# imulki/serenade

Hardware: AMD Instinct MI355X
Metric: mel frames/sec converted (UNet ODE + vocoder), 80x1024 (higher is better)
Workload: dtype f32

## Files before the change

### include/serenade_hip.h

```cpp
#ifndef SERENADE_HIP_H
#define SERENADE_HIP_H

#include <stdint.h>

#ifdef __cplusplus
extern "C" {
#endif

#define SRN_ABI_VERSION 4
#define SRN_MAX_TAPS 16

enum { SRN_ACT_NONE = 0, SRN_ACT_LEAKY = 1, SRN_ACT_SILU = 2, SRN_ACT_MISH = 3 };
enum { SRN_RES_NONE = 0, SRN_RES_ADD = 1, SRN_RES_AXPY = 2 };
enum {
  SRN_POST_NONE = 0,
  SRN_POST_DIV = 1,
  SRN_POST_TANH = 2,
  SRN_POST_RELU = 3,
  SRN_POST_LEAKY = 4,
  SRN_POST_GELU = 5
};
enum {
  SRN_PREC_FP32 = 0,
  SRN_PREC_BF16X3 = 1,
  SRN_PREC_BF16X6 = 2
};
enum {
  SRN_ROUTE_AUTO = 0,
  SRN_ROUTE_TILED = 1,
  SRN_ROUTE_HALO = 2,
  SRN_ROUTE_GENERIC = 3,
  SRN_ROUTE_STRIP = 4,
  SRN_ROUTE_FAST_FP32 = 5
};
enum {
  SRN_FAMILY_GENERIC = 0,
  SRN_FAMILY_F32 = 1,
  SRN_FAMILY_FAST = 2,
  SRN_FAMILY_HALO = 3,
  SRN_FAMILY_STRIP = 4
};

typedef struct SrnConvParams {
  int32_t n_batch;
  int32_t n_head;
  int32_t T_in, T_out;
  int32_t C_in;
  int32_t C_in0;
  int32_t C_w;
  int32_t N;
  int32_t N_out;
  int32_t n_taps;
  int32_t tap_off[SRN_MAX_TAPS];
  int32_t in_stride;
  int32_t pad_reflect;
  int32_t w_nmajor;
  int32_t pro_act;
  float pro_slope;
  float alpha;
  float beta;
  int32_t geglu;
  int32_t res_mode;
  int32_t post;
  float post_div;
  int32_t out_t_stride, out_t_off;
  int32_t tile;
  const float* in0; int64_t in0_bs, in0_hs; int32_t ld_in0;
  const float* in1; int64_t in1_bs; int32_t ld_in1;
  const float* w;   int64_t w_bs, w_hs; int32_t ldw;
  const float* bias;
  const int32_t* len_in;
  const int32_t* len_out;
  const float* res;  int64_t res_bs, res_hs; int32_t ld_res;
  const float* res2; int64_t res2_bs; int32_t ld_res2;
  float* out; int64_t out_bs, out_hs; int32_t ld_out;
  int32_t precision;
  int32_t route;
  void* ws; int64_t ws_bytes;
  const void* w_hi; const void* w_lo;
  float* gn_partials;
  float* out_tr; int64_t out_tr_bs; int32_t ld_out_tr; int32_t out_tr_col0;
} SrnConvParams;

int srn_abi_version(void);
const char* srn_last_error(void);

int srn_conv_gemm(const SrnConvParams* p, void* stream);
int64_t srn_conv_gemm_workspace_bytes(const SrnConvParams* p);
int srn_conv_gemm_route(const SrnConvParams* p, int32_t out[3]);
#define SRN_FORM_FIELDS 9
int srn_conv_gemm_forms(int32_t* rows, int capacity);

int srn_gn_mish_apply(const float* x, const float* gn_partials, const float* gamma, const float* beta,
                      const float* time_bias, int64_t time_bias_bs, const int32_t* lens, float* y, int B, int T,
                      int C, int groups, float eps, int valid_stats, void* stream);

int srn_resblock_tail(const float* c2, const float* gn_partials, const float* gamma, const float* beta,
                      const int32_t* lens, const float* r, const float* scale, const float* shift, int64_t ld_ss,
                      float* y, int B, int T, int C, int groups, float gn_eps, float ln_eps, int valid_stats,
                      void* stream);

int srn_resblock_tail_ln(const float* c2, const float* gn_partials, const float* gamma, const float* beta,
                         const int32_t* lens, const float* r, const float* scale, const float* shift, int64_t ld_ss,
                         float* y, int B, int T, int C, int groups, float gn_eps, float ln_eps, int valid_stats,
                         const float* ln2_gamma, const float* ln2_beta, float* y2, float ln2_eps, void* stream);

int srn_layernorm(const float* x, const float* gamma, const float* beta, float* y, int64_t rows, int C, float eps,
                  void* stream);

int srn_softmax_rows(float* s, const int32_t* lens, int Z, int n_head, int L, int ld, void* stream);

int srn_sinusoidal_emb(const float* t, float* out, int n, int dim, int ld, float scale, void* stream);

int srn_copy_channels(const float* src, int64_t src_bs, int ld_src, int sc0, float* dst, int64_t dst_bs, int ld_dst,
                      int dc0, int B, int T, int C, void* stream);

int srn_scatter_rows(const float* src, int64_t src_bs, int ld_src, float* dst, int64_t dst_bs, int ld_dst, int dc0,
                     const int32_t* row_off, const int32_t* n_rows, int B, int T, int C, void* stream);

int srn_transpose_ct(const float* src, float* dst, int B, int R, int Cc, int64_t src_bs, int ld_src, int64_t dst_bs,
                     int ld_dst, void* stream);
#define SRN_TR_LIST_MAX 40
typedef struct SrnTransposeList {
  int32_t n;
  int32_t pad_;
  const float* src[SRN_TR_LIST_MAX];
  float* dst[SRN_TR_LIST_MAX];
  int64_t src_bs[SRN_TR_LIST_MAX], dst_bs[SRN_TR_LIST_MAX];
  int32_t B[SRN_TR_LIST_MAX], R[SRN_TR_LIST_MAX], Cc[SRN_TR_LIST_MAX];
  int32_t ld_src[SRN_TR_LIST_MAX], ld_dst[SRN_TR_LIST_MAX];
  int32_t first_block[SRN_TR_LIST_MAX + 1];
} SrnTransposeList;
int srn_transpose_multi(const SrnTransposeList* list, void* stream);

int srn_renorm(const float* x, const float* trg_scale, const float* trg_mean, const float* voc_mean,
               const float* voc_scale, float* y, int64_t rows, int C, void* stream);

int srn_out_conv_tanh(const float* x, const float* w, const float* bias, float* y, int B, int T, int C, int k,
                      float slope, void* stream);

typedef struct SrnResUnitParams {
  int32_t n_batch, T, C;
  int32_t k, dilation;
  float slope;
  const float* x; int64_t x_bs;
  const float* w1; const float* b1; const float* w2; const float* b2;
  const void* w1_hi; const void* w2_hi;
  const float* res2; int64_t res2_bs;
  float post_div;
  float* out; int64_t out_bs;
  int32_t precision;
  int32_t route;
} SrnResUnitParams;
enum { SRN_RESUNIT_ROUTE_SHARED = 1 };


int srn_hifigan_resunit(const SrnResUnitParams* p, void* stream);
enum { SRN_RESUNIT_FORM_F32 = 0, SRN_RESUNIT_FORM_SHARED_F32 = 1, SRN_RESUNIT_FORM_BF16X3 = 2 };
int srn_hifigan_resunit_route(const SrnResUnitParams* p, int32_t out[3]);

int srn_pd_gather(const float* x, const float* d, float* out, int B, int T, int C, float dilation, float slope,
                  void* stream);

int srn_gru_recur_last(const float* gi, const float* w_hh_t, const float* b_hh, float* h, int B, int T, int H,
                       void* stream);

int srn_style_token_attention_kv(const float* ref, const float* wq_t, const float* bq, const float* k, const float* v,
                                 const float* wo_t, const float* bo, float* out, int B, int Dq, int n_tok, int F,
                                 int n_head, void* stream);

int srn_pad_signal(const float* x, float* out, int B, int n, int pad, int ld, int mode, void* stream);
int srn_logmel(const float* spec, const float* mel_t, float* out, int64_t frames, int n_bins, int ld, int n_mels,
               float eps, int log_mode, void* stream);
int srn_loudness(const float* spec, const float* a_weight_db, uint32_t* gmax_ws, float* out, int B, int frames,
                 int n_bins, int ld, float amin, float top_db, float add_eps, void* stream);
int srn_pad_ragged_zero(const float* x, int64_t x_bs, const int32_t* lens, float* out, int B, int n, int pad, int ld,
                        void* stream);
int srn_logmel_ragged(const float* spec, const float* mel_t, const int32_t* frames, float* out, int B, int T,
                      int n_bins, int ld, int n_mels, float eps, int log_mode, void* stream);
int srn_loudness_ragged(const float* spec, const float* a_weight_db, const int32_t* frames, uint32_t* gmax_ws,
                        float* out, int B, int T, int n_bins, int ld, float amin, float top_db, float add_eps,
                        void* stream);

int srn_rowln_fwd(const float* x, const float* m, int64_t m_bs, const float* a, int64_t a_bs, float* y, int B, int T,
                  int C, float eps, void* stream);
int srn_rowln_bwd(const float* x, const float* dy, const float* m, int64_t m_bs, float* dx, float* partial, int B, int T,
                  int C, float eps, void* stream);
int srn_rowln_chunks(int T);
int srn_gn_mish_bwd_partial(const float* h, const float* dy, const float* mean, const float* rstd, const float* gamma,
                            const float* beta, const int32_t* lens, float* partial, int B, int T, int C, int groups,
                            void* stream);
int srn_gn_mish_bwd_apply(const float* h, const float* dy, const float* mean, const float* rstd, const float* gamma,
                          const float* beta, const float* gsum, const int32_t* lens, float* dh, int B, int T, int C,
                          int groups, void* stream);
int srn_gn_chunks(int T);
int srn_gn_stats(const float* partials, float* mean, float* rstd, int B, int T, int C, int groups, float eps,
                 void* stream);
int srn_chunk_colsum(const float* partial, const float* gamma, float* col, float* gsum, int B, int n_chunk, int C,
                     int groups, void* stream);
int srn_colsum(const float* x, float* partial, float* out, int B, int64_t R, int N, int ld, void* stream);
int srn_colsum_chunks(int64_t R);
int srn_softmax_bwd(const float* p, float* dp, int64_t rows, int L, int ld, float scale, void* stream);
int srn_geglu_fwd(const float* hg, float* a, int64_t rows, int inner, void* stream);
int srn_geglu_bwd(const float* hg, const float* da, float* dhg, int64_t rows, int inner, void* stream);
int srn_adamw(float* p, const float* g, float* m, float* v, int64_t n, float lr, float beta1, float beta2, float eps,
              float weight_decay, int step, float grad_scale, void* stream);
int srn_adamw_dyn(float* p, const float* g, float* m, float* v, int64_t n, float beta1, float beta2, float eps,
                  float weight_decay, const float* dyn, void* stream);
int srn_sumsq(const float* g, int64_t n, double* partial, void* stream);
int srn_dot(const float* a, const float* b, int64_t n, double* partial, void* stream);
#define SRN_COPY_LIST_MAX 160
typedef struct SrnCopyList {
  int32_t n;
  int32_t pad_;
  const void* src[SRN_COPY_LIST_MAX];
  int64_t off[SRN_COPY_LIST_MAX];
  int64_t len[SRN_COPY_LIST_MAX];
} SrnCopyList;
int srn_multi_copy(const SrnCopyList* list, float* dst, void* stream);
int srn_sumsq_blocks(int64_t n);
int srn_weight_norm_fwd(const float* v, const float* g, float* w_packed, float* wd, float* inv_norm, int N, int C, int k,
                        void* stream);
int srn_weight_norm_bwd(const float* dw_packed, const float* v, const float* g, const float* inv_norm, float* dv,
                        float* dg, int N, int C, int k, void* stream);

typedef struct SrnWorldParams {
  int32_t n_batch, max_frames;
  int32_t fs, fft_size;
  const double* x; int64_t x_bs; const int32_t* x_len;
  const double* f0; const double* t; int64_t f_bs;
  const int32_t* n_frames;
  const double* twiddle;
  double q1, f0_floor;
  double threshold;
  double unvoiced_db;
  const double* band_window; int32_t band_window_len;
  int32_t n_bands;
  double* out0; int64_t out0_bs; int32_t ld_out0;
  double* out1; int64_t out1_bs; int32_t ld_out1;
} SrnWorldParams;
int srn_world_cheaptrick(const SrnWorldParams* p, void* stream);
int srn_world_d4c(const SrnWorldParams* p, void* stream);
int srn_world_project(const double* in, int64_t rows, int K, int ld_in, const double* mat_t, int n_out, int take_log,
                      double* out, int ld_out, void* stream);
int srn_world_pack_features(const double* a, int na, const double* b, int nb, const double* mean, const double* scale,
                            float* out, int64_t rows, int ld_out, void* stream);
int srn_wave_to_f64(const float* wave, double* out, int64_t n, int pcm16, void* stream);
int srn_f0_match_length(const double* in, int64_t in_bs, const int32_t* n_in, double* out, int64_t out_bs,
// ... 136 lines not shown
```

### serenade_amd/_lib.py

```python
import collections
import ctypes
import os
from ctypes import POINTER, c_char_p, c_double, c_float, c_int, c_int32, c_int64, c_void_p

_HERE = os.path.dirname(os.path.abspath(__file__))
LIB_PATH = os.environ.get("SERENADE_AMD_LIB") or os.path.join(_HERE, "libserenade_hip.so")

SRN_MAX_TAPS = 16
ACT_NONE, ACT_LEAKY, ACT_SILU, ACT_MISH = 0, 1, 2, 3
RES_NONE, RES_ADD, RES_AXPY = 0, 1, 2
POST_NONE, POST_DIV, POST_TANH, POST_RELU, POST_LEAKY, POST_GELU = 0, 1, 2, 3, 4, 5
PREC_FP32, PREC_BF16X3, PREC_BF16X6 = 0, 1, 2
ROUTE_AUTO, ROUTE_TILED, ROUTE_HALO, ROUTE_GENERIC, ROUTE_STRIP, ROUTE_FAST_FP32 = 0, 1, 2, 3, 4, 5
FAMILY_GENERIC, FAMILY_F32, FAMILY_FAST, FAMILY_HALO, FAMILY_STRIP = 0, 1, 2, 3, 4
RESUNIT_ROUTE_SHARED = 1
TN_ROUTE_GENERAL = 1
RESUNIT_FORM_F32, RESUNIT_FORM_SHARED_F32, RESUNIT_FORM_BF16X3 = 0, 1, 2


class SrnConvParams(ctypes.Structure):
    _fields_ = [
        ("n_batch", c_int32), ("n_head", c_int32), ("T_in", c_int32), ("T_out", c_int32),
        ("C_in", c_int32), ("C_in0", c_int32), ("C_w", c_int32), ("N", c_int32), ("N_out", c_int32),
        ("n_taps", c_int32), ("tap_off", c_int32 * SRN_MAX_TAPS), ("in_stride", c_int32),
        ("pad_reflect", c_int32), ("w_nmajor", c_int32), ("pro_act", c_int32), ("pro_slope", c_float),
        ("alpha", c_float), ("beta", c_float), ("geglu", c_int32), ("res_mode", c_int32), ("post", c_int32), ("post_div", c_float),
        ("out_t_stride", c_int32), ("out_t_off", c_int32), ("tile", c_int32),
        ("in0", c_void_p), ("in0_bs", c_int64), ("in0_hs", c_int64), ("ld_in0", c_int32),
        ("in1", c_void_p), ("in1_bs", c_int64), ("ld_in1", c_int32),
        ("w", c_void_p), ("w_bs", c_int64), ("w_hs", c_int64), ("ldw", c_int32),
        ("bias", c_void_p), ("len_in", c_void_p), ("len_out", c_void_p),
        ("res", c_void_p), ("res_bs", c_int64), ("res_hs", c_int64), ("ld_res", c_int32),
        ("res2", c_void_p), ("res2_bs", c_int64), ("ld_res2", c_int32),
        ("out", c_void_p), ("out_bs", c_int64), ("out_hs", c_int64), ("ld_out", c_int32),
        ("precision", c_int32), ("route", c_int32), ("ws", c_void_p), ("ws_bytes", c_int64),
        ("w_hi", c_void_p), ("w_lo", c_void_p), ("gn_partials", c_void_p),
        ("out_tr", c_void_p), ("out_tr_bs", c_int64), ("ld_out_tr", c_int32), ("out_tr_col0", c_int32),
    ]


class SrnResUnitParams(ctypes.Structure):
    _fields_ = [
        ("n_batch", c_int32), ("T", c_int32), ("C", c_int32), ("k", c_int32), ("dilation", c_int32),
        ("slope", c_float), ("x", c_void_p), ("x_bs", c_int64),
        ("w1", c_void_p), ("b1", c_void_p), ("w2", c_void_p), ("b2", c_void_p),
        ("w1_hi", c_void_p), ("w2_hi", c_void_p), ("res2", c_void_p), ("res2_bs", c_int64),
        ("post_div", c_float), ("out", c_void_p), ("out_bs", c_int64), ("precision", c_int32), ("route", c_int32),
    ]


SRN_COPY_LIST_MAX = 160


class SrnCopyList(ctypes.Structure):
    _fields_ = [("n", c_int32), ("pad_", c_int32), ("src", c_void_p * SRN_COPY_LIST_MAX),
                ("off", c_int64 * SRN_COPY_LIST_MAX), ("len", c_int64 * SRN_COPY_LIST_MAX)]


class SrnWorldParams(ctypes.Structure):
    _fields_ = [
        ("n_batch", c_int32), ("max_frames", c_int32), ("fs", c_int32), ("fft_size", c_int32),
        ("x", c_void_p), ("x_bs", c_int64), ("x_len", c_void_p),
        ("f0", c_void_p), ("t", c_void_p), ("f_bs", c_int64), ("n_frames", c_void_p), ("twiddle", c_void_p),
        ("q1", c_double), ("f0_floor", c_double), ("threshold", c_double), ("unvoiced_db", c_double),
        ("band_window", c_void_p), ("band_window_len", c_int32), ("n_bands", c_int32),
        ("out0", c_void_p), ("out0_bs", c_int64), ("ld_out0", c_int32),
        ("out1", c_void_p), ("out1_bs", c_int64), ("ld_out1", c_int32),
    ]


SRN_TR_LIST_MAX = 40


class SrnTransposeList(ctypes.Structure):
    _fields_ = [("n", c_int32), ("pad_", c_int32), ("src", c_void_p * SRN_TR_LIST_MAX), ("dst", c_void_p * SRN_TR_LIST_MAX),
                ("src_bs", c_int64 * SRN_TR_LIST_MAX), ("dst_bs", c_int64 * SRN_TR_LIST_MAX),
                ("B", c_int32 * SRN_TR_LIST_MAX), ("R", c_int32 * SRN_TR_LIST_MAX), ("Cc", c_int32 * SRN_TR_LIST_MAX),
                ("ld_src", c_int32 * SRN_TR_LIST_MAX), ("ld_dst", c_int32 * SRN_TR_LIST_MAX),
                ("first_block", c_int32 * (SRN_TR_LIST_MAX + 1))]


class SrnTnGemmParams(ctypes.Structure):
    _fields_ = [
        ("n_batch", c_int32), ("n_head", c_int32), ("n_items", c_int32), ("T_a", c_int32), ("T_b", c_int32),
        ("stride", c_int32), ("n_shifts", c_int32), ("shift", c_int32 * SRN_MAX_TAPS), ("M", c_int32), ("N", c_int32),
        ("a", c_void_p), ("a_bs", c_int64), ("a_hs", c_int64), ("a_is", c_int64), ("lda", c_int32),
        ("b", c_void_p), ("b_bs", c_int64), ("b_hs", c_int64), ("b_is", c_int64), ("ldb", c_int32),
        ("out", c_void_p), ("out_bs", c_int64), ("out_hs", c_int64), ("ldc", c_int32),
        ("alpha", c_float), ("ws", c_void_p), ("ws_bytes", c_int64),
        ("n_inner", c_int32), ("a_is2", c_int64), ("b_is2", c_int64), ("len_b", c_void_p), ("colsum", c_void_p),
        ("route", c_int32),
    ]


class SrnExcitationParams(ctypes.Structure):
    _fields_ = [
        ("n_batch", c_int32), ("max_frames", c_int32), ("fs", c_int32), ("hop", c_int32),
        ("f0", c_void_p), ("df_f0", c_void_p), ("f_bs", c_int64), ("n_frames", c_void_p), ("phase_ws", c_void_p),
        ("noise", c_void_p), ("sine", c_void_p), ("sine_amp", c_float), ("noise_amp", c_float), ("n_df", c_int32),
        ("dfs", c_void_p * 4), ("df_upsample", c_int32 * 4), ("dense_factors", c_double * 4),
    ]


_P = c_void_p
_SIGS = {
    "srn_abi_version": (c_int, []),
    "srn_last_error": (c_char_p, []),
    "srn_conv_gemm": (c_int, [POINTER(SrnConvParams), _P]),
    "srn_conv_gemm_workspace_bytes": (c_int64, [POINTER(SrnConvParams)]),
    "srn_conv_gemm_route": (c_int, [POINTER(SrnConvParams), POINTER(c_int32)]),
    "srn_conv_gemm_forms": (c_int, [POINTER(c_int32), c_int]),
    "srn_hifigan_resunit": (c_int, [POINTER(SrnResUnitParams), _P]),
    "srn_hifigan_resunit_route": (c_int, [POINTER(SrnResUnitParams), POINTER(c_int32)]),
    "srn_gn_mish_apply": (c_int, [_P, _P, _P, _P, _P, c_int64, _P, _P, c_int, c_int, c_int, c_int, c_float, c_int, _P]),
    "srn_resblock_tail": (c_int, [_P, _P, _P, _P, _P, _P, _P, _P, c_int64, _P, c_int, c_int, c_int, c_int,
                                  c_float, c_float, c_int, _P]),
    "srn_resblock_tail_ln": (c_int, [_P, _P, _P, _P, _P, _P, _P, _P, c_int64, _P, c_int, c_int, c_int, c_int,
                                     c_float, c_float, c_int, _P, _P, _P, c_float, _P]),
    "srn_scatter_rows": (c_int, [_P, c_int64, c_int, _P, c_int64, c_int, c_int, _P, _P, c_int, c_int, c_int, _P]),
    "srn_layernorm": (c_int, [_P, _P, _P, _P, c_int64, c_int, c_float, _P]),
    "srn_softmax_rows": (c_int, [_P, _P, c_int, c_int, c_int, c_int, _P]),
    "srn_sinusoidal_emb": (c_int, [_P, _P, c_int, c_int, c_int, c_float, _P]),
    "srn_copy_channels": (c_int, [_P, c_int64, c_int, c_int, _P, c_int64, c_int, c_int, c_int, c_int, c_int, _P]),
    "srn_transpose_ct": (c_int, [_P, _P, c_int, c_int, c_int, c_int64, c_int, c_int64, c_int, _P]),
    "srn_transpose_multi": (c_int, [POINTER(SrnTransposeList), _P]),
    "srn_weight_norm_fwd": (c_int, [_P, _P, _P, _P, _P, c_int, c_int, c_int, _P]),
    "srn_weight_norm_bwd": (c_int, [_P, _P, _P, _P, _P, _P, c_int, c_int, c_int, _P]),
    "srn_renorm": (c_int, [_P, _P, _P, _P, _P, _P, c_int64, c_int, _P]),
    "srn_out_conv_tanh": (c_int, [_P, _P, _P, _P, c_int, c_int, c_int, c_int, c_float, _P]),
    "srn_pd_gather": (c_int, [_P, _P, _P, c_int, c_int, c_int, c_float, c_float, _P]),
    "srn_pad_signal": (c_int, [_P, _P, c_int, c_int, c_int, c_int, c_int, _P]),
    "srn_logmel": (c_int, [_P, _P, _P, c_int64, c_int, c_int, c_int, c_float, c_int, _P]),
    "srn_loudness": (c_int, [_P, _P, _P, _P, c_int, c_int, c_int, c_int, c_float, c_float, c_float, _P]),
    "srn_pad_ragged_zero": (c_int, [_P, c_int64, _P, _P, c_int, c_int, c_int, c_int, _P]),
    "srn_logmel_ragged": (c_int, [_P, _P, _P, _P, c_int, c_int, c_int, c_int, c_int, c_float, c_int, _P]),
    "srn_loudness_ragged": (c_int, [_P, _P, _P, _P, _P, c_int, c_int, c_int, c_int, c_float, c_float, c_float, _P]),
    "srn_gru_recur_last": (c_int, [_P, _P, _P, _P, c_int, c_int, c_int, _P]),
    "srn_style_token_attention_kv": (c_int, [_P] * 8 + [c_int] * 5 + [_P]),
    "srn_rowln_fwd": (c_int, [_P, _P, c_int64, _P, c_int64, _P, c_int, c_int, c_int, c_float, _P]),
    "srn_rowln_bwd": (c_int, [_P, _P, _P, c_int64, _P, _P, c_int, c_int, c_int, c_float, _P]),
    "srn_rowln_chunks": (c_int, [c_int]),
    "srn_gn_mish_bwd_partial": (c_int, [_P] * 8 + [c_int] * 4 + [_P]),
    "srn_gn_mish_bwd_apply": (c_int, [_P] * 9 + [c_int] * 4 + [_P]),
    "srn_gn_chunks": (c_int, [c_int]),
    "srn_gn_stats": (c_int, [_P, _P, _P, c_int, c_int, c_int, c_int, c_float, _P]),
    "srn_chunk_colsum": (c_int, [_P, _P, _P, _P, c_int, c_int, c_int, c_int, _P]),
    "srn_colsum": (c_int, [_P, _P, _P, c_int, c_int64, c_int, c_int, _P]),
    "srn_colsum_chunks": (c_int, [c_int64]),
    "srn_softmax_bwd": (c_int, [_P, _P, c_int64, c_int, c_int, c_float, _P]),
    "srn_geglu_fwd": (c_int, [_P, _P, c_int64, c_int, _P]),
    "srn_geglu_bwd": (c_int, [_P, _P, _P, c_int64, c_int, _P]),
    "srn_adamw": (c_int, [_P, _P, _P, _P, c_int64, c_float, c_float, c_float, c_float, c_float, c_int, c_float, _P]),
    "srn_adamw_dyn": (c_int, [_P, _P, _P, _P, c_int64, c_float, c_float, c_float, c_float, _P, _P]),
    "srn_sumsq": (c_int, [_P, c_int64, _P, _P]),
    "srn_dot": (c_int, [_P, _P, c_int64, _P, _P]),
    "srn_multi_copy": (c_int, [POINTER(SrnCopyList), _P, _P]),
    "srn_sumsq_blocks": (c_int, [c_int64]),
    "srn_bn_chunks": (c_int, [c_int64]),
    "srn_bn_relu_fwd": (c_int, [_P] * 8 + [c_int64, c_int, c_float, c_float, _P]),
    "srn_bn_relu_bwd": (c_int, [_P] * 8 + [c_int64, c_int, _P]),
    "srn_im2col_s2": (c_int, [_P, _P] + [c_int] * 5 + [_P]),
    "srn_col2im_s2": (c_int, [_P, _P] + [c_int] * 5 + [_P]),
    "srn_gru_train_fwd": (c_int, [_P] * 5 + [c_int] * 3 + [_P]),
    "srn_gru_train_bwd": (c_int, [_P] * 6 + [c_int] * 3 + [_P]),
    "srn_token_attn_fwd": (c_int, [_P] * 5 + [c_int] * 4 + [_P]),
    "srn_token_attn_bwd": (c_int, [_P] * 8 + [c_int] * 4 + [_P]),
    "srn_tn_gemm": (c_int, [POINTER(SrnTnGemmParams), _P]),
    "srn_tn_gemm_workspace_bytes": (c_int64, [POINTER(SrnTnGemmParams)]),
    "srn_tn_gemm_route": (c_int, [POINTER(SrnTnGemmParams), POINTER(c_int32)]),
    "srn_world_cheaptrick": (c_int, [POINTER(SrnWorldParams), _P]),
    "srn_world_d4c": (c_int, [POINTER(SrnWorldParams), _P]),
    "srn_world_project": (c_int, [_P, c_int64, c_int, c_int, _P, c_int, c_int, _P, c_int, _P]),
    "srn_world_pack_features": (c_int, [_P, c_int, _P, c_int, _P, _P, _P, c_int64, c_int, _P]),
    "srn_wave_to_f64": (c_int, [_P, _P, c_int64, c_int, _P]),
    "srn_f0_match_length": (c_int, [_P, c_int64, _P, _P, c_int64, _P, c_int, c_int, _P]),
    "srn_cont_f0": (c_int, [_P, c_int64, _P, _P, _P, _P, c_int, _P]),
    "srn_sifigan_excitation": (c_int, [POINTER(SrnExcitationParams), _P]),
    "srn_frame_stats_chunks": (c_int, [c_int]),
    "srn_cvec_conv0": (c_int, [_P, c_int64, c_int, _P, _P, _P, _P] + [c_int] * 5 + [_P]),
    "srn_channel_norm_gelu": (c_int, [_P, _P, c_int, _P, _P, _P, _P, _P, c_int, c_int, c_int, c_float, _P]),
    "srn_posconv_gelu_res": (c_int, [_P] * 5 + [c_int] * 6 + [_P]),
    "srn_pad_ragged": (c_int, [_P, c_int64, _P, _P, c_int, c_int, c_int, c_int, _P]),
    "srn_mel_db": (c_int, [_P, c_int, c_int, _P, _P, _P, _P, c_int, c_int, c_int, c_int, c_float, c_float, _P]),
    "srn_trans_conv0": (c_int, [_P, c_int64, c_int, _P, _P, _P, _P] + [c_int] * 5 + [_P]),
    "srn_trans_pool": (c_int, [_P, _P, _P] + [c_int] * 7 + [_P]),
    "srn_bilstm_slices": (c_int, [c_int]),
    "srn_bilstm_recur": (c_int, [_P, c_int64, c_int, _P, _P, _P, c_int64, c_int, c_int, c_int, c_int, _P]),
    "srn_pyin_observe": (c_int, [_P, c_int64] + [_P] * 9 + [c_int] * 10 + [c_double] * 3 + [c_int, _P]),
    "srn_pyin_viterbi": (c_int, [_P] * 6 + [c_double] * 2 + [c_int] + [_P] * 4 + [c_int] * 4 + [_P]),
    "srn_harvest_decimate": (c_int, [_P, c_int, c_int64, _P, _P, _P, c_int64, _P, c_int64] + [c_int] * 4 + [_P]),
    "srn_harvest_channels": (c_int, [_P, c_int64] + [_P] * 6 + [c_int, _P, c_int64, _P] + [c_int] * 6
                             + [c_double] * 3 + [_P]),
    "srn_harvest_candidates": (c_int, [_P] * 4 + [c_int] * 4 + [_P]),
    "srn_harvest_refine": (c_int, [_P, c_int64] + [_P] * 5 + [c_int] * 3 + [c_double] * 3 + [_P]),
    "srn_harvest_contour": (c_int, [_P] * 9 + [c_int64, _P, c_int, _P, _P, c_int64] + [c_int] * 5 + [c_double, _P]),
    "srn_resample": (c_int, [_P, c_int, c_int64, _P, _P, _P, _P, c_int64] + [c_int] * 7 + [_P]),
    "srn_trim_bounds": (c_int, [_P, c_int, c_int64, _P, _P, _P] + [c_int] * 5 + [c_double, _P]),
    "srn_wave_window": (c_int, [_P, c_int, c_int64, _P, _P, c_int, _P, c_int64, c_int, c_int, _P]),
    "srn_col_moments": (c_int, [_P, _P, c_int64] + [_P] * 5 + [c_int, c_int, _P]),
    "srn_scale_collate": (c_int, [_P, _P, c_int64, _P, _P, _P, c_int, _P] + [c_int] * 4 + [_P]),
}

EXPORTS = tuple(_SIGS)

_lib = None


def lib():
    global _lib
    if _lib is None:
        if not os.path.exists(LIB_PATH):
            raise RuntimeError(
                f"{LIB_PATH} not found: build it with `python -m serenade_amd.build` "
                "(hipcc --offload-arch=gfx950). There is no CPU fallback.")
        h = ctypes.CDLL(LIB_PATH)
        for name, (res, args) in _SIGS.items():
            fn = getattr(h, name)
            fn.restype = res
            fn.argtypes = args
        if h.srn_abi_version() != 4:
            raise RuntimeError("libserenade_hip.so ABI version mismatch")
        _lib = h
    return _lib


def check(rc, what=""):
    if rc != 0:
        msg = lib().srn_last_error().decode("utf-8", "replace")
        raise RuntimeError(f"libserenade_hip {what} failed (rc={rc}): {msg}")


ConvForm = collections.namedtuple("ConvForm", "family tile precision nmajor kslices bm bn wn stages")


def conv_forms():
    k = len(ConvForm._fields)
    n = lib().srn_conv_gemm_forms(None, 0)
    rows = (c_int32 * (n * k))()
    assert lib().srn_conv_gemm_forms(rows, n) == n
    return [ConvForm(*rows[i * k:(i + 1) * k]) for i in range(n)]
```

### serenade_amd/csrc/norm_act.hip

```cpp
#include "common.h"
#include "conv_common.h"
#include "row_common.h"

namespace {

__device__ __forceinline__ void group_stats(const float* __restrict__ partials, int b, int T, int C, int groups,
                                            float eps, float* s_mean, float* s_rstd, int n_rows) {
  gn_group_stats(partials, b, T, C, groups, eps, n_rows,
                 [&](int g, float mean, float rstd) { s_mean[g] = mean, s_rstd[g] = rstd; });
  __syncthreads();
}

constexpr int GN_ROWS = 8;
constexpr int SMALL_GRID = 512;
constexpr int GN_PRE = 4;

__global__ __launch_bounds__(256) void gn_mish_apply_kernel(const float* __restrict__ x,
                                                            const float* __restrict__ partials,
                                                            const float* __restrict__ gamma,
                                                            const float* __restrict__ beta,
                                                            const float* __restrict__ time_bias,
                                                            const int32_t* __restrict__ lens, float* __restrict__ y,
                                                            int T, int C, int groups, float eps, int64_t tb_bs,
                                                            int valid_stats, int rows_per_wg) {
  __shared__ float s_mean[64], s_rstd[64];
  const int b = blockIdx.y;
  const int r0 = blockIdx.x * rows_per_wg;
  if (time_bias) time_bias += (int64_t)b * tb_bs;
  const int len = lens ? min(lens[b], T) : T;
  const int c4n = C / 4;
  const int cpg = C / groups;
  const int rows = min(rows_per_wg, T - r0);
  const int total = rows * c4n;
  const int64_t base = ((int64_t)b * T + r0) * C;
  float4 pre[GN_PRE];
#pragma unroll
  for (int k = 0; k < GN_PRE; ++k) {
    const int idx = threadIdx.x + 256 * k;
    pre[k] = make_float4(0.f, 0.f, 0.f, 0.f);
    if (idx < total) {
      const int r = idx / c4n;
      if (r0 + r < len) pre[k] = *reinterpret_cast<const float4*>(x + base + (int64_t)r * C + (idx - r * c4n) * 4);
    }
  }
  group_stats(partials, b, T, C, groups, eps, s_mean, s_rstd, valid_stats ? len : T);
  auto one = [&](const int idx, const float4 v) {
    const int r = idx / c4n;
    const int c = (idx - r * c4n) * 4;
    float4 o = make_float4(0.f, 0.f, 0.f, 0.f);
    if (r0 + r < len) {
      const float4 ga = *reinterpret_cast<const float4*>(gamma + c);
      const float4 be = *reinterpret_cast<const float4*>(beta + c);
      const int g = c / cpg;
      o = gn_mish4(v, s_mean[g], s_rstd[g], ga, be);
      if (time_bias) {
        const float4 tb = *reinterpret_cast<const float4*>(time_bias + c);
        o.x += tb.x;
        o.y += tb.y;
        o.z += tb.z;
        o.w += tb.w;
      }
    }
    *reinterpret_cast<float4*>(y + base + (int64_t)r * C + c) = o;
  };
#pragma unroll
  for (int k = 0; k < GN_PRE; ++k)
    if ((int)threadIdx.x + 256 * k < total) one(threadIdx.x + 256 * k, pre[k]);
  for (int idx = threadIdx.x + 256 * GN_PRE; idx < total; idx += 256) {
    const int r = idx / c4n;
    float4 v = make_float4(0.f, 0.f, 0.f, 0.f);
    if (r0 + r < len) v = *reinterpret_cast<const float4*>(x + base + (int64_t)r * C + (idx - r * c4n) * 4);
    one(idx, v);
  }
}

constexpr int TAIL_ROWS = 8;

__global__ __launch_bounds__(256) void resblock_tail_kernel(
    const float* __restrict__ c2, const float* __restrict__ partials, const float* __restrict__ gamma,
    const float* __restrict__ beta, const int32_t* __restrict__ lens, const float* __restrict__ rres,
    const float* __restrict__ scale, const float* __restrict__ shift, int64_t ld_ss, float* __restrict__ y, int T,
    int C, int groups, float gn_eps, float ln_eps, int valid_stats, const float* __restrict__ ln2_gamma,
    const float* __restrict__ ln2_beta, float* __restrict__ y2, float ln2_eps, int rows_per_wg) {
  __shared__ float s_mean[64], s_rstd[64];
  const int b = blockIdx.y;
  const int r0 = blockIdx.x * rows_per_wg;
  const int len = lens ? min(lens[b], T) : T;
  const int wave = threadIdx.x >> 6, lane = threadIdx.x & 63;
  const int c4n = C / 4;
  const int cpg = C / groups;
  const float inv_c = 1.0f / (float)C;
  const int r_end = min(r0 + rows_per_wg, T);
  float4 xin[MAXV], rin[MAXV];
  auto fetch = [&](const int r) {
    const int64_t row = ((int64_t)b * T + r) * C;
#pragma unroll
    for (int i = 0; i < MAXV; ++i) {
      const int c4 = lane + 64 * i;
      xin[i] = rin[i] = make_float4(0.f, 0.f, 0.f, 0.f);
      if (c4 < c4n) {
        rin[i] = *reinterpret_cast<const float4*>(rres + row + c4 * 4);
        if (r < len) xin[i] = *reinterpret_cast<const float4*>(c2 + row + c4 * 4);
      }
    }
  };
  if (r0 + wave < r_end) fetch(r0 + wave);
  group_stats(partials, b, T, C, groups, gn_eps, s_mean, s_rstd, valid_stats ? len : T);
  for (int r = r0 + wave; r < r_end; r += 4) {
    if (r != r0 + wave) fetch(r);
    const int64_t row = ((int64_t)b * T + r) * C;
    const bool valid = r < len;
    float4 v[MAXV];
#pragma unroll
    for (int i = 0; i < MAXV; ++i) {
      const int c4 = lane + 64 * i;
      v[i] = make_float4(0.f, 0.f, 0.f, 0.f);
      if (c4 < c4n) {
        const int c = c4 * 4;
        const float4 rr = rin[i];
        float4 o = make_float4(0.f, 0.f, 0.f, 0.f);
        if (valid) {
          const float4 ga = *reinterpret_cast<const float4*>(gamma + c);
          const float4 be = *reinterpret_cast<const float4*>(beta + c);
          const int g = c / cpg;
          o = gn_mish4(xin[i], s_mean[g], s_rstd[g], ga, be);
        }
        v[i] = make_float4(o.x + rr.x, o.y + rr.y, o.z + rr.z, o.w + rr.w);
      }
    }
    const float mean = row_sum(v, lane, c4n) * inv_c;
    const float stdv = sqrtf(row_sqdev(v, mean, lane, c4n) * inv_c + ln_eps);
    row_norm_affine_store<true>(v, mean, stdv, scale + (int64_t)b * ld_ss, shift + (int64_t)b * ld_ss, y + row, lane,
                                c4n);
    if (y2 != nullptr) row_layernorm_store(v, ln2_eps, ln2_gamma, ln2_beta, y2 + row, lane, c4n, inv_c);
  }
}

__global__ __launch_bounds__(256) void layernorm_kernel(const float* __restrict__ x, const float* __restrict__ gamma,
                                                        const float* __restrict__ beta, float* __restrict__ y,
                                                        int64_t rows, int C, float eps) {
  const int wave = threadIdx.x >> 6, lane = threadIdx.x & 63;
  const int c4n = C / 4;
  const float inv_c = 1.0f / (float)C;
  for (int64_t r = (int64_t)blockIdx.x * 4 + wave; r < rows; r += (int64_t)gridDim.x * 4) {
    float4 v[MAXV];
    row_load(x + r * C, v, lane, c4n);
    row_layernorm_store(v, eps, gamma, beta, y + r * C, lane, c4n, inv_c);
  }
}

template <int NV>
__global__ __launch_bounds__(256) void softmax_rows_kernel(float* __restrict__ s, const int32_t* __restrict__ lens,
                                                           int64_t n_rows, int n_head, int L, int ld) {
  const int wave = threadIdx.x >> 6, lane = threadIdx.x & 63;
  const int64_t r = (int64_t)blockIdx.x * 4 + wave;
  if (r >= n_rows) return;
  const int z = (int)(r / L);
  int len = L;
  if (lens) len = min(lens[z / n_head], L);
  float* row = s + r * ld;
  const int ld4 = ld / 4;
  float4 v[NV];
  float mx = -INFINITY;
#pragma unroll
  for (int i = 0; i < NV; ++i) {
    const int c4 = lane + 64 * i;
    v[i] = make_float4(-INFINITY, -INFINITY, -INFINITY, -INFINITY);
    if (c4 < ld4) {
      const float4 t = *reinterpret_cast<const float4*>(row + c4 * 4);
      const int c = c4 * 4;
      if (c + 0 < len) v[i].x = t.x;
      if (c + 1 < len) v[i].y = t.y;
      if (c + 2 < len) v[i].z = t.z;
      if (c + 3 < len) v[i].w = t.w;
      mx = fmaxf(mx, fmaxf(fmaxf(v[i].x, v[i].y), fmaxf(v[i].z, v[i].w)));
    }
  }
  mx = wave_max(mx);
  float sum = 0.f;
#pragma unroll
  for (int i = 0; i < NV; ++i) {
    if (lane + 64 * i < ld4) {
      v[i].x = expf(v[i].x - mx);
      v[i].y = expf(v[i].y - mx);
      v[i].z = expf(v[i].z - mx);
      v[i].w = expf(v[i].w - mx);
      sum += (v[i].x + v[i].y) + (v[i].z + v[i].w);
    }
  }
  sum = wave_sum(sum);
#pragma unroll
  for (int i = 0; i < NV; ++i) {
    const int c4 = lane + 64 * i;
    if (c4 < ld4) {
      float4 o;
      o.x = v[i].x / sum;
      o.y = v[i].y / sum;
      o.z = v[i].z / sum;
      o.w = v[i].w / sum;
      *reinterpret_cast<float4*>(row + c4 * 4) = o;
    }
  }
}

__global__ void sinusoidal_emb_kernel(const float* __restrict__ t, float* __restrict__ out, int n, int dim,
                                      int ld, float scale) {
  const int half = dim / 2;
  const int idx = blockIdx.x * blockDim.x + threadIdx.x;
  if (idx >= n * half) return;
  const int i = idx / half, k = idx - i * half;
  const float emb = logf(10000.0f) / (float)(half - 1);
  const float f = expf((float)k * -emb);
  const float arg = scale * t[i] * f;
  out[(int64_t)i * ld + k] = sinf(arg);
  out[(int64_t)i * ld + half + k] = cosf(arg);
}

__global__ void copy_channels_kernel(const float* __restrict__ src, int64_t src_bs, int ld_src, int sc0,
                                     float* __restrict__ dst, int64_t dst_bs, int ld_dst, int dc0, int T, int C) {
  const int b = blockIdx.y;
  const int64_t total = (int64_t)T * C;
  for (int64_t idx = (int64_t)blockIdx.x * blockDim.x + threadIdx.x; idx < total;
       idx += (int64_t)gridDim.x * blockDim.x) {
    const int t = (int)(idx / C), c = (int)(idx - (int64_t)t * C);
    dst[(int64_t)b * dst_bs + (int64_t)t * ld_dst + dc0 + c] = src[(int64_t)b * src_bs + (int64_t)t * ld_src + sc0 + c];
  }
}

__global__ void scatter_rows_kernel(const float* __restrict__ src, int64_t src_bs, int ld_src,
                                    float* __restrict__ dst, int64_t dst_bs, int ld_dst, int dc0,
                                    const int32_t* __restrict__ row_off, const int32_t* __restrict__ n_rows, int T,
                                    int C) {
  const int b = blockIdx.y;
  const int off = row_off ? row_off[b] : 0;
  const int64_t total = (int64_t)min(n_rows ? n_rows[b] : T, T) * C;
  for (int64_t idx = (int64_t)blockIdx.x * blockDim.x + threadIdx.x; idx < total;
       idx += (int64_t)gridDim.x * blockDim.x) {
    const int t = (int)(idx / C), c = (int)(idx - (int64_t)t * C);
    dst[(int64_t)b * dst_bs + (int64_t)(off + t) * ld_dst + dc0 + c] = src[(int64_t)b * src_bs + (int64_t)t * ld_src + c];
  }
}

__global__ __launch_bounds__(256) void transpose_kernel(const float* __restrict__ src, float* __restrict__ dst, int R,
                                                        int Cc, int64_t src_bs, int ld_src, int64_t dst_bs,
                                                        int ld_dst) {
  __shared__ float tile[32][33];
  const int b = blockIdx.z;
  const int r0 = blockIdx.y * 32, c0 = blockIdx.x * 32;
  const int tx = threadIdx.x & 31, ty = threadIdx.x >> 5;
  for (int i = ty; i < 32; i += 8) {
    const int r = r0 + i, c = c0 + tx;
    tile[i][tx] = (r < R && c < Cc) ? src[(int64_t)b * src_bs + (int64_t)r * ld_src + c] : 0.f;
  }
  __syncthreads();
  for (int i = ty; i < 32; i += 8) {
    const int c = c0 + i, r = r0 + tx;
    if (c < Cc && r < R) dst[(int64_t)b * dst_bs + (int64_t)c * ld_dst + r] = tile[tx][i];
  }
}

__global__ __launch_bounds__(256) void transpose_multi_kernel(const SrnTransposeList L) {
  __shared__ float tile[32][33];
  int e = 0;
  while (e + 1 < L.n && (int)blockIdx.x >= L.first_block[e + 1]) ++e;
  const int blk = blockIdx.x - L.first_block[e];
  const float* __restrict__ src = L.src[e];
  float* __restrict__ dst = L.dst[e];
  const int R = L.R[e], Cc = L.Cc[e], ld_src = L.ld_src[e], ld_dst = L.ld_dst[e];
  const int64_t src_bs = L.src_bs[e], dst_bs = L.dst_bs[e];
  if (R < 16 || Cc < 16) {
    const int64_t per_b = (int64_t)R * Cc, total = per_b * L.B[e];
    for (int i = 0; i < 4; ++i) {
      const int64_t idx = (int64_t)blk * 1024 + i * 256 + threadIdx.x;
      if (idx >= total) return;
      const int b = (int)(idx / per_b);
      const int rem = (int)(idx - (int64_t)b * per_b);
      const int c = rem / R, r = rem - c * R;
      dst[b * dst_bs + (int64_t)c * ld_dst + r] = src[b * src_bs + (int64_t)r * ld_src + c];
    }
    return;
  }
  const int tc = (Cc + 31) / 32, tr = (R + 31) / 32;
  const int b = blk / (tc * tr), t = blk - b * tc * tr;
  const int r0 = (t / tc) * 32, c0 = (t % tc) * 32;
  const int tx = threadIdx.x & 31, ty = threadIdx.x >> 5;
  for (int i = ty; i < 32; i += 8) {
    const int r = r0 + i, c = c0 + tx;
    tile[i][tx] = (r < R && c < Cc) ? src[b * src_bs + (int64_t)r * ld_src + c] : 0.f;
  }
  __syncthreads();
  for (int i = ty; i < 32; i += 8) {
    const int c = c0 + i, r = r0 + tx;
    if (c < Cc && r < R) dst[b * dst_bs + (int64_t)c * ld_dst + r] = tile[tx][i];
  }
}

__global__ void renorm_kernel(const float* __restrict__ x, const float* __restrict__ ts, const float* __restrict__ tm,
                              const float* __restrict__ vm, const float* __restrict__ vs, float* __restrict__ y,
                              int64_t total, int C) {
  for (int64_t idx = (int64_t)blockIdx.x * blockDim.x + threadIdx.x; idx < total;
       idx += (int64_t)gridDim.x * blockDim.x) {
    const int c = (int)(idx % C);
    float v = x[idx];
    if (ts) v = v * ts[c] + tm[c];
    y[idx] = (v - vm[c]) / vs[c];
  }
}

constexpr int OC_BT = 256;
template <int K, int CC>
__global__ __launch_bounds__(256) void out_conv_tanh_kernel(const float* __restrict__ x, const float* __restrict__ w,
                                                            const float* __restrict__ bias, float* __restrict__ y,
                                                            int T, float slope) {
  constexpr int PITCH = CC + 4;
  constexpr int ROWS = OC_BT + K - 1;
  __shared__ __attribute__((aligned(16))) float sx[ROWS * PITCH];
  __shared__ __attribute__((aligned(16))) float sw[K * CC];
  const int b = blockIdx.y;
  const int t0 = blockIdx.x * OC_BT;
  const float* xb = x + (int64_t)b * T * CC;
  for (int i = threadIdx.x; i < K * CC; i += 256) sw[i] = w[i];
  constexpr int C4 = CC / 4;
  for (int i = threadIdx.x; i < ROWS * C4; i += 256) {
    const int r = i / C4, c4 = i - r * C4;
    const int ti = t0 + r - (K - 1) / 2;
    float4 v = make_float4(0.f, 0.f, 0.f, 0.f);
    if (ti >= 0 && ti < T) v = leaky4(*reinterpret_cast<const float4*>(xb + (int64_t)ti * CC + c4 * 4), slope);
    *reinterpret_cast<float4*>(sx + r * PITCH + c4 * 4) = v;
  }
  __syncthreads();
  const int t = t0 + threadIdx.x;
  if (t >= T) return;
  float acc = bias[0];
#pragma unroll
  for (int j = 0; j < K; ++j) {
    const float* row = sx + (threadIdx.x + j) * PITCH;
#pragma unroll
    for (int c4 = 0; c4 < C4; ++c4) {
      const float4 v = *reinterpret_cast<const float4*>(row + c4 * 4);
      const float4 ww = *reinterpret_cast<const float4*>(sw + j * CC + c4 * 4);
      acc = fmaf(v.x, ww.x, acc);
      acc = fmaf(v.y, ww.y, acc);
      acc = fmaf(v.z, ww.z, acc);
      acc = fmaf(v.w, ww.w, acc);
    }
  }
  y[(int64_t)b * T + t] = tanhf(acc);
}

__global__ __launch_bounds__(256) void out_conv_tanh_generic(const float* __restrict__ x, const float* __restrict__ w,
                                                             const float* __restrict__ bias, float* __restrict__ y,
                                                             int T, int C, int K, float slope) {
  const int b = blockIdx.y;
  const int t = blockIdx.x * 256 + threadIdx.x;
  if (t >= T) return;
  const float* xb = x + (int64_t)b * T * C;
  float acc = bias[0];
  for (int j = 0; j < K; ++j) {
    const int ti = t + j - (K - 1) / 2;
    if (ti < 0 || ti >= T) continue;
    for (int c = 0; c < C; ++c) {
      float v = xb[(int64_t)ti * C + c];
      v = v > 0.f ? v : v * slope;
      acc = fmaf(v, w[j * C + c], acc);
    }
  }
  y[(int64_t)b * T + t] = tanhf(acc);
}

}

extern "C" int srn_gn_mish_apply(const float* x, const float* gn_partials, const float* gamma, const float* beta,
                                 const float* time_bias, int64_t time_bias_bs, const int32_t* lens, float* y, int B,
                                 int T, int C, int groups, float eps, int valid_stats, void* stream) {
  SRN_CHECK_ARG(x && gn_partials && gamma && beta && y, "gn_mish_apply: null pointer");
  SRN_CHECK_ARG(!valid_stats || lens, "gn_mish_apply: valid_stats needs lens");
  SRN_CHECK_ARG(B > 0 && T > 0 && C > 0 && groups > 0 && groups <= 64 && C % groups == 0 && (C / groups) % 32 == 0,
                "gn_mish_apply: need (C / groups) %% 32 == 0 (C=%d groups=%d)", C, groups);
  const int rows_per_wg = (int64_t)B * ((T + GN_ROWS - 1) / GN_ROWS) < SMALL_GRID ? GN_ROWS / 2 : GN_ROWS;
  dim3 grid((T + rows_per_wg - 1) / rows_per_wg, B);
  hipLaunchKernelGGL(gn_mish_apply_kernel, grid, dim3(256), 0, (hipStream_t)stream, x, gn_partials, gamma, beta,
                     time_bias, lens, y, T, C, groups, eps, time_bias_bs, valid_stats, rows_per_wg);
  SRN_CHECK_LAUNCH();
  return 0;
}

static int resblock_tail_launch(const char* name, const float* c2, const float* gn_partials, const float* gamma,
                                const float* beta, const int32_t* lens, const float* r, const float* scale,
                                const float* shift, int64_t ld_ss, float* y, int B, int T, int C, int groups, float gn_eps,
                                float ln_eps, int valid_stats, const float* ln2_gamma, const float* ln2_beta, float* y2,
                                float ln2_eps, void* stream) {
  SRN_CHECK_ARG(c2 && gn_partials && gamma && beta && r && scale && shift && y, "%s: null pointer", name);
  SRN_CHECK_ARG(!valid_stats || lens, "%s: valid_stats needs lens", name);
  SRN_CHECK_ARG(B > 0 && T > 0 && C > 0 && C % 4 == 0 && C <= 256 * MAXV, "%s: C=%d unsupported", name, C);
  SRN_CHECK_ARG(groups > 0 && groups <= 64 && C % groups == 0 && (C / groups) % 32 == 0,
                "%s: need (C / groups) %% 32 == 0", name);
  const int rows_per_wg = (int64_t)B * ((T + TAIL_ROWS - 1) / TAIL_ROWS) < SMALL_GRID ? TAIL_ROWS / 2 : TAIL_ROWS;
  dim3 grid((T + rows_per_wg - 1) / rows_per_wg, B);
  hipLaunchKernelGGL(resblock_tail_kernel, grid, dim3(256), 0, (hipStream_t)stream, c2, gn_partials, gamma, beta,
                     lens, r, scale, shift, ld_ss, y, T, C, groups, gn_eps, ln_eps, valid_stats, ln2_gamma, ln2_beta,
                     y2, ln2_eps, rows_per_wg);
  SRN_CHECK_LAUNCH();
  return 0;
}

extern "C" int srn_resblock_tail(const float* c2, const float* gn_partials, const float* gamma, const float* beta,
                                 const int32_t* lens, const float* r, const float* scale, const float* shift,
                                 int64_t ld_ss, float* y, int B, int T, int C, int groups, float gn_eps,
                                 float ln_eps, int valid_stats, void* stream) {
  return resblock_tail_launch("resblock_tail", c2, gn_partials, gamma, beta, lens, r, scale, shift, ld_ss, y, B, T, C,
                              groups, gn_eps, ln_eps, valid_stats, nullptr, nullptr, nullptr, 0.f, stream);
}

extern "C" int srn_resblock_tail_ln(const float* c2, const float* gn_partials, const float* gamma, const float* beta,
                                    const int32_t* lens, const float* r, const float* scale, const float* shift,
                                    int64_t ld_ss, float* y, int B, int T, int C, int groups, float gn_eps,
                                    float ln_eps, int valid_stats, const float* ln2_gamma, const float* ln2_beta,
                                    float* y2, float ln2_eps, void* stream) {
  SRN_CHECK_ARG(ln2_gamma && ln2_beta && y2, "resblock_tail_ln: null pointer");
  return resblock_tail_launch("resblock_tail_ln", c2, gn_partials, gamma, beta, lens, r, scale, shift, ld_ss, y, B, T,
                              C, groups, gn_eps, ln_eps, valid_stats, ln2_gamma, ln2_beta, y2, ln2_eps, stream);
}

extern "C" int srn_layernorm(const float* x, const float* gamma, const float* beta, float* y, int64_t rows, int C,
                             float eps, void* stream) {
  SRN_CHECK_ARG(x && gamma && beta && y, "layernorm: null pointer");
  SRN_CHECK_ARG(rows > 0 && C > 0 && C % 4 == 0 && C <= 256 * MAXV, "layernorm: C=%d unsupported", C);
  int64_t blocks = (rows + 3) / 4;
  if (blocks > 65536) blocks = 65536;
  hipLaunchKernelGGL(layernorm_kernel, dim3((unsigned)blocks), dim3(256), 0, (hipStream_t)stream, x, gamma, beta, y,
                     rows, C, eps);
  SRN_CHECK_LAUNCH();
  return 0;
}

extern "C" int srn_softmax_rows(float* s, const int32_t* lens, int Z, int n_head, int L, int ld, void* stream) {
  SRN_CHECK_ARG(s != nullptr && Z > 0 && n_head > 0 && L > 0 && ld >= L && ld % 4 == 0, "softmax_rows: bad args");
  const int64_t rows = (int64_t)Z * L;
  const unsigned blocks = (unsigned)((rows + 3) / 4);
  const int nv = (ld / 4 + 63) / 64;
  hipStream_t st = (hipStream_t)stream;
  if (nv <= 2) hipLaunchKernelGGL(softmax_rows_kernel<2>, dim3(blocks), dim3(256), 0, st, s, lens, rows, n_head, L, ld);
  else if (nv <= 4) hipLaunchKernelGGL(softmax_rows_kernel<4>, dim3(blocks), dim3(256), 0, st, s, lens, rows, n_head, L, ld);
  else if (nv <= 8) hipLaunchKernelGGL(softmax_rows_kernel<8>, dim3(blocks), dim3(256), 0, st, s, lens, rows, n_head, L, ld);
  else if (nv <= 12) hipLaunchKernelGGL(softmax_rows_kernel<12>, dim3(blocks), dim3(256), 0, st, s, lens, rows, n_head, L, ld);
  else if (nv <= 20) hipLaunchKernelGGL(softmax_rows_kernel<20>, dim3(blocks), dim3(256), 0, st, s, lens, rows, n_head, L, ld);
  else if (nv <= 36) hipLaunchKernelGGL(softmax_rows_kernel<36>, dim3(blocks), dim3(256), 0, st, s, lens, rows, n_head, L, ld);
  else {
    srn_set_error("softmax_rows: ld=%d too long (max 9216)", ld);
    return -1;
  }
  SRN_CHECK_LAUNCH();
  return 0;
}

extern "C" int srn_sinusoidal_emb(const float* t, float* out, int n, int dim, int ld, float scale, void* stream) {
  SRN_CHECK_ARG(t && out && n > 0 && dim > 2 && dim % 2 == 0 && ld >= dim, "sinusoidal_emb: bad args");
  const int total = n * (dim / 2);
  hipLaunchKernelGGL(sinusoidal_emb_kernel, dim3((total + 255) / 256), dim3(256), 0, (hipStream_t)stream, t, out, n,
                     dim, ld, scale);
  SRN_CHECK_LAUNCH();
  return 0;
}

extern "C" int srn_copy_channels(const float* src, int64_t src_bs, int ld_src, int sc0, float* dst, int64_t dst_bs,
                                 int ld_dst, int dc0, int B, int T, int C, void* stream) {
  SRN_CHECK_ARG(src && dst && B > 0 && T > 0 && C > 0, "copy_channels: bad args");
  int64_t blocks = ((int64_t)T * C + 255) / 256;
  if (blocks > 4096) blocks = 4096;
  hipLaunchKernelGGL(copy_channels_kernel, dim3((unsigned)blocks, B), dim3(256), 0, (hipStream_t)stream, src, src_bs,
                     ld_src, sc0, dst, dst_bs, ld_dst, dc0, T, C);
  SRN_CHECK_LAUNCH();
  return 0;
}

extern "C" int srn_scatter_rows(const float* src, int64_t src_bs, int ld_src, float* dst, int64_t dst_bs, int ld_dst,
                                int dc0, const int32_t* row_off, const int32_t* n_rows, int B, int T, int C,
                                void* stream) {
  SRN_CHECK_ARG(src && dst && B > 0 && T > 0 && C > 0, "scatter_rows: bad args");
  int64_t blocks = ((int64_t)T * C + 255) / 256;
  if (blocks > 1024) blocks = 1024;
  hipLaunchKernelGGL(scatter_rows_kernel, dim3((unsigned)blocks, B), dim3(256), 0, (hipStream_t)stream, src, src_bs,
                     ld_src, dst, dst_bs, ld_dst, dc0, row_off, n_rows, T, C);
  SRN_CHECK_LAUNCH();
  return 0;
}

extern "C" int srn_transpose_ct(const float* src, float* dst, int B, int R, int Cc, int64_t src_bs, int ld_src,
                                int64_t dst_bs, int ld_dst, void* stream) {
  SRN_CHECK_ARG(src && dst && B > 0 && R > 0 && Cc > 0, "transpose_ct: bad args");
  dim3 grid((Cc + 31) / 32, (R + 31) / 32, B);
  hipLaunchKernelGGL(transpose_kernel, grid, dim3(256), 0, (hipStream_t)stream, src, dst, R, Cc, src_bs, ld_src,
                     dst_bs, ld_dst);
  SRN_CHECK_LAUNCH();
  return 0;
}

extern "C" int srn_transpose_multi(const SrnTransposeList* list, void* stream) {
  SRN_CHECK_ARG(list != nullptr && list->n > 0 && list->n <= SRN_TR_LIST_MAX, "transpose_multi: bad list");
  SrnTransposeList L = *list;
  int64_t blocks = 0;
  for (int e = 0; e < L.n; ++e) {
    SRN_CHECK_ARG(L.src[e] && L.dst[e] && L.B[e] > 0 && L.R[e] > 0 && L.Cc[e] > 0 && L.ld_src[e] >= L.Cc[e] &&
                      L.ld_dst[e] >= L.R[e],
                  "transpose_multi: entry %d: bad pointers / sizes / leading dimensions", e);
    L.first_block[e] = (int32_t)blocks;
    if (L.R[e] < 16 || L.Cc[e] < 16) blocks += ((int64_t)L.B[e] * L.R[e] * L.Cc[e] + 1023) / 1024;
    else blocks += (int64_t)L.B[e] * ((L.R[e] + 31) / 32) * ((L.Cc[e] + 31) / 32);
    SRN_CHECK_ARG(blocks < (1ll << 31), "transpose_multi: grid too large");
  }
  L.first_block[L.n] = (int32_t)blocks;
  hipLaunchKernelGGL(transpose_multi_kernel, dim3((unsigned)blocks), dim3(256), 0, (hipStream_t)stream, L);
  SRN_CHECK_LAUNCH();
  return 0;
}

extern "C" int srn_renorm(const float* x, const float* trg_scale, const float* trg_mean, const float* voc_mean,
                          const float* voc_scale, float* y, int64_t rows, int C, void* stream) {
  SRN_CHECK_ARG(x && voc_mean && voc_scale && y && rows > 0 && C > 0, "renorm: bad args");
  SRN_CHECK_ARG((trg_scale == nullptr) == (trg_mean == nullptr), "renorm: trg_scale/trg_mean must come together");
  int64_t blocks = (rows * C + 255) / 256;
  if (blocks > 4096) blocks = 4096;
  hipLaunchKernelGGL(renorm_kernel, dim3((unsigned)blocks), dim3(256), 0, (hipStream_t)stream, x, trg_scale, trg_mean,
                     voc_mean, voc_scale, y, rows * C, C);
  SRN_CHECK_LAUNCH();
  return 0;
}

extern "C" int srn_out_conv_tanh(const float* x, const float* w, const float* bias, float* y, int B, int T, int C,
                                 int k, float slope, void* stream) {
  SRN_CHECK_ARG(x && w && bias && y && B > 0 && T > 0 && C > 0 && k > 0 && k % 2 == 1 && k <= 16,
                "out_conv_tanh: bad args");
// ... 54 lines not shown
```

Before: 62560.

## Size GN-Mish grid to CU count and double-buffer row walk

The GroupNorm+Mish apply kernel now launches roughly two workgroups per CU, each walking many rows, instead of one workgroup per eight rows. The inner loop is software-pipelined with two register buffers, so the next block of float4 loads is issued while the current one is normalised and stored. Per-channel gamma/beta/time-bias and group stats are cached in registers and advanced incrementally instead of being reloaded with a divide per element. Each workgroup also recomputes group stats only once per many rows, which cuts that redundant work, but the larger per-workgroup items risk tail imbalance and higher register pressure.

```diff
diff --git a/include/serenade_hip.h b/include/serenade_hip.h
--- a/include/serenade_hip.h
+++ b/include/serenade_hip.h
@@ -94,6 +94,7 @@
 int srn_gn_mish_apply(const float* x, const float* gn_partials, const float* gamma, const float* beta,
                       const float* time_bias, int64_t time_bias_bs, const int32_t* lens, float* y, int B, int T,
                       int C, int groups, float eps, int valid_stats, void* stream);
+int srn_gn_walk_rows(int B, int T);
 
 int srn_resblock_tail(const float* c2, const float* gn_partials, const float* gamma, const float* beta,
                       const int32_t* lens, const float* r, const float* scale, const float* shift, int64_t ld_ss,
diff --git a/serenade_amd/_lib.py b/serenade_amd/_lib.py
--- a/serenade_amd/_lib.py
+++ b/serenade_amd/_lib.py
@@ -113,6 +113,7 @@
     "srn_hifigan_resunit": (c_int, [POINTER(SrnResUnitParams), _P]),
     "srn_hifigan_resunit_route": (c_int, [POINTER(SrnResUnitParams), POINTER(c_int32)]),
     "srn_gn_mish_apply": (c_int, [_P, _P, _P, _P, _P, c_int64, _P, _P, c_int, c_int, c_int, c_int, c_float, c_int, _P]),
+    "srn_gn_walk_rows": (c_int, [c_int, c_int]),
     "srn_resblock_tail": (c_int, [_P, _P, _P, _P, _P, _P, _P, _P, c_int64, _P, c_int, c_int, c_int, c_int,
                                   c_float, c_float, c_int, _P]),
     "srn_resblock_tail_ln": (c_int, [_P, _P, _P, _P, _P, _P, _P, _P, c_int64, _P, c_int, c_int, c_int, c_int,
diff --git a/serenade_amd/csrc/norm_act.hip b/serenade_amd/csrc/norm_act.hip
--- a/serenade_amd/csrc/norm_act.hip
+++ b/serenade_amd/csrc/norm_act.hip
@@ -14,6 +14,14 @@
 constexpr int GN_ROWS = 8;
 constexpr int SMALL_GRID = 512;
 constexpr int GN_PRE = 4;
+constexpr int GN_BLOCK = 256 * GN_PRE;
+constexpr int GN_WG_PER_CU = 2;
+
+int gn_walk_rows(int B, int T) {
+  if ((int64_t)B * ((T + GN_ROWS - 1) / GN_ROWS) < SMALL_GRID) return GN_ROWS / 2;
+  const int nx = max(1, SRN_NUM_CUS * GN_WG_PER_CU / B);
+  return (T + nx - 1) / nx;
+}
 
 __global__ __launch_bounds__(256) void gn_mish_apply_kernel(const float* __restrict__ x,
                                                             const float* __restrict__ partials,
@@ -32,45 +40,82 @@
   const int cpg = C / groups;
   const int rows = min(rows_per_wg, T - r0);
   const int total = rows * c4n;
+  const int live = max(0, min(len - r0, rows)) * c4n;
   const int64_t base = ((int64_t)b * T + r0) * C;
-  float4 pre[GN_PRE];
-#pragma unroll
-  for (int k = 0; k < GN_PRE; ++k) {
-    const int idx = threadIdx.x + 256 * k;
-    pre[k] = make_float4(0.f, 0.f, 0.f, 0.f);
-    if (idx < total) {
-      const int r = idx / c4n;
-      if (r0 + r < len) pre[k] = *reinterpret_cast<const float4*>(x + base + (int64_t)r * C + (idx - r * c4n) * 4);
-    }
-  }
+  const float4* __restrict__ x4 = reinterpret_cast<const float4*>(x + base);
+  float4* __restrict__ y4 = reinterpret_cast<float4*>(y + base);
+  const int step = GN_BLOCK % c4n;
+  int c4[GN_PRE];
+  float4 ga[GN_PRE], be[GN_PRE], tb[GN_PRE];
+  float mu[GN_PRE], rs[GN_PRE];
+  auto fetch = [&](float4(&d)[GN_PRE], const int i0) {
+#pragma unroll
+    for (int k = 0; k < GN_PRE; ++k) {
+      const int idx = i0 + threadIdx.x + 256 * k;
+      d[k] = make_float4(0.f, 0.f, 0.f, 0.f);
+      if (idx < live) d[k] = x4[idx];
+    }
+  };
+  auto channel_params = [&]() {
+#pragma unroll
+    for (int k = 0; k < GN_PRE; ++k) {
+      ga[k] = *reinterpret_cast<const float4*>(gamma + c4[k] * 4);
+      be[k] = *reinterpret_cast<const float4*>(beta + c4[k] * 4);
+      if (time_bias) tb[k] = *reinterpret_cast<const float4*>(time_bias + c4[k] * 4);
+    }
+  };
+  auto group_params = [&]() {
+#pragma unroll
+    for (int k = 0; k < GN_PRE; ++k) {
+      const int g = c4[k] * 4 / cpg;
+      mu[k] = s_mean[g], rs[k] = s_rstd[g];
+    }
+  };
+  auto emit = [&](const float4(&d)[GN_PRE], const int i0) {
+#pragma unroll
+    for (int k = 0; k < GN_PRE; ++k) {
+      const int idx = i0 + threadIdx.x + 256 * k;
+      if (idx < total) {
+        float4 o = make_float4(0.f, 0.f, 0.f, 0.f);
+        if (idx < live) {
+          o = gn_mish4(d[k], mu[k], rs[k], ga[k], be[k]);
+          if (time_bias) {
+            o.x += tb[k].x;
+            o.y += tb[k].y;
+            o.z += tb[k].z;
+            o.w += tb[k].w;
+          }
+        }
+        y4[idx] = o;
+      }
+    }
+  };
+  float4 d0[GN_PRE], d1[GN_PRE];
+  fetch(d0, 0);
+#pragma unroll
+  for (int k = 0; k < GN_PRE; ++k) c4[k] = (threadIdx.x + 256 * k) % c4n;
+  channel_params();
   group_stats(partials, b, T, C, groups, eps, s_mean, s_rstd, valid_stats ? len : T);
-  auto one = [&](const int idx, const float4 v) {
-    const int r = idx / c4n;
-    const int c = (idx - r * c4n) * 4;
-    float4 o = make_float4(0.f, 0.f, 0.f, 0.f);
-    if (r0 + r < len) {
-      const float4 ga = *reinterpret_cast<const float4*>(gamma + c);
-      const float4 be = *reinterpret_cast<const float4*>(beta + c);
-      const int g = c / cpg;
-      o = gn_mish4(v, s_mean[g], s_rstd[g], ga, be);
-      if (time_bias) {
-        const float4 tb = *reinterpret_cast<const float4*>(time_bias + c);
-        o.x += tb.x;
-        o.y += tb.y;
-        o.z += tb.z;
-        o.w += tb.w;
-      }
-    }
-    *reinterpret_cast<float4*>(y + base + (int64_t)r * C + c) = o;
+  group_params();
+  auto advance = [&]() {
+    if (step == 0) return;
+#pragma unroll
+    for (int k = 0; k < GN_PRE; ++k) {
+      c4[k] += step;
+      if (c4[k] >= c4n) c4[k] -= c4n;
+    }
+    channel_params();
+    group_params();
   };
-#pragma unroll
-  for (int k = 0; k < GN_PRE; ++k)
-    if ((int)threadIdx.x + 256 * k < total) one(threadIdx.x + 256 * k, pre[k]);
-  for (int idx = threadIdx.x + 256 * GN_PRE; idx < total; idx += 256) {
-    const int r = idx / c4n;
-    float4 v = make_float4(0.f, 0.f, 0.f, 0.f);
-    if (r0 + r < len) v = *reinterpret_cast<const float4*>(x + base + (int64_t)r * C + (idx - r * c4n) * 4);
-    one(idx, v);
+  for (int i0 = 0;;) {
+    fetch(d1, i0 + GN_BLOCK);
+    emit(d0, i0);
+    if ((i0 += GN_BLOCK) >= total) break;
+    advance();
+    fetch(d0, i0 + GN_BLOCK);
+    emit(d1, i0);
+    if ((i0 += GN_BLOCK) >= total) break;
+    advance();
   }
 }
 
@@ -370,6 +415,8 @@
 
 }
 
+extern "C" int srn_gn_walk_rows(int B, int T) { return B > 0 && T > 0 ? gn_walk_rows(B, T) : 0; }
+
 extern "C" int srn_gn_mish_apply(const float* x, const float* gn_partials, const float* gamma, const float* beta,
                                  const float* time_bias, int64_t time_bias_bs, const int32_t* lens, float* y, int B,
                                  int T, int C, int groups, float eps, int valid_stats, void* stream) {
@@ -377,7 +424,8 @@
   SRN_CHECK_ARG(!valid_stats || lens, "gn_mish_apply: valid_stats needs lens");
   SRN_CHECK_ARG(B > 0 && T > 0 && C > 0 && groups > 0 && groups <= 64 && C % groups == 0 && (C / groups) % 32 == 0,
                 "gn_mish_apply: need (C / groups) %% 32 == 0 (C=%d groups=%d)", C, groups);
-  const int rows_per_wg = (int64_t)B * ((T + GN_ROWS - 1) / GN_ROWS) < SMALL_GRID ? GN_ROWS / 2 : GN_ROWS;
+  const int rows_per_wg = gn_walk_rows(B, T);
+  SRN_CHECK_ARG((int64_t)rows_per_wg * (C / 4) + GN_BLOCK < (1ll << 31), "gn_mish_apply: item too large");
   dim3 grid((T + rows_per_wg - 1) / rows_per_wg, B);
   hipLaunchKernelGGL(gn_mish_apply_kernel, grid, dim3(256), 0, (hipStream_t)stream, x, gn_partials, gamma, beta,
                      time_bias, lens, y, T, C, groups, eps, time_bias_bs, valid_stats, rows_per_wg);
```

Result: no change. 62600, median of 3 (+0.1%).
